# mhalushka/miRge3.0

Hardware: AMD Instinct MI355X
Metric: M reads/s through full annotation cascade; per-class counts bit-exact vs ref (higher is better)
Workload: dtype u64

## Files before the change

### mirge3.0_amd/csrc/kernels_collapse.hpp

```cpp
#pragma once
template <int W>
__device__ __forceinline__ bool same_read(const GroupView<W>& g, uint32_t a, const MirgeRead<W>& r) {
    if (g.len[a] != (uint8_t)r.len) return false;
    bool eq = true;
#pragma unroll
    for (int w = 0; w < W; w++) {
        eq &= g.seq[(size_t)w * g.n + a] == r.w[w];
        if (g.nmask) eq &= g.nmask[(size_t)w * g.n + a] == r.nm[w];
    }
    return eq;
}

template <int W>
__global__ void k_collapse_insert(GroupView<W> g, uint32_t* __restrict__ rep, uint32_t* __restrict__ firstj,
                                  uint32_t* __restrict__ cnt, uint32_t* __restrict__ slot_of,
                                  uint32_t mask, const int32_t* __restrict__ sample_ids,
                                  const uint32_t* __restrict__ orig, uint32_t base, int32_t S, uint32_t j_lo, uint32_t j_hi,
                                  const uint32_t* __restrict__ weight) {
    __shared__ unsigned long long c_key[MIRGE_CELL_CACHE];
    __shared__ uint32_t c_min[MIRGE_CELL_CACHE];
    __shared__ uint32_t c_cnt[MIRGE_CELL_CACHE];
    for (uint32_t i = threadIdx.x; i < MIRGE_CELL_CACHE; i += blockDim.x) { c_key[i] = 0ull; c_min[i] = 0xFFFFFFFFu; c_cnt[i] = 0; }
    __syncthreads();
    for (uint32_t j = j_lo + blockIdx.x * blockDim.x + threadIdx.x; j < j_hi; j += gridDim.x * blockDim.x) {
// ... 4 lines not shown
        for (int w = 1; w < W; w++) h = mirge_mix64(h ^ r.w[w]);
#pragma unroll
        for (int w = 0; w < W; w++) h ^= mirge_mix64(r.nm[w] + 0x9e3779b97f4a7c15ull * (w + 1));
        uint32_t s = (uint32_t)(h >> 20) & mask;
        while (true) {
            uint32_t cur = rep[s];
            if (cur == MIRGE_EMPTY) cur = atomicCAS(&rep[s], MIRGE_EMPTY, j);
            if (cur == MIRGE_EMPTY || cur == j || same_read<W>(g, cur, r)) break;
            s = (s + 1) & mask;
        }
        slot_of[j] = s;
        const uint32_t hidx = orig ? orig[j] : base + j;
        const int32_t sid = sample_ids ? sample_ids[hidx] : 0;
        const uint32_t wgt = weight ? weight[hidx] : 1u;
        const unsigned long long cell = (unsigned long long)s * (unsigned)S + (unsigned)sid + 1ull;
        uint32_t cs = (uint32_t)(mirge_mix64(cell) >> 11) & (MIRGE_CELL_CACHE - 1);
        bool cached = false;
        for (int t = 0; t < 4; t++) {
            unsigned long long cur = c_key[cs];
            if (cur == 0ull) cur = atomicCAS(&c_key[cs], 0ull, cell);
            if (cur == 0ull || cur == cell) {
                atomicMin(&c_min[cs], j);
                atomicAdd(&c_cnt[cs], wgt);
                cached = true;
                break;
            }
            cs = (cs + 1) & (MIRGE_CELL_CACHE - 1);
        }
        if (!cached) {
            atomicMin(&firstj[s], j);
            atomicAdd(&cnt[(size_t)s * S + sid], wgt);
        }
    }
    __syncthreads();
    for (uint32_t i = threadIdx.x; i < MIRGE_CELL_CACHE; i += blockDim.x) {
        const unsigned long long cell = c_key[i];
        if (cell == 0ull) continue;
        const unsigned long long lin = cell - 1ull;
        atomicMin(&firstj[lin / (unsigned)S], c_min[i]);
        atomicAdd(&cnt[lin], c_cnt[i]);
    }
}

struct KeySlot {
    unsigned long long key;
    uint32_t first_inv;
    uint32_t cnt;
};

__global__ void k_collapse_insert_key(GroupView<1> g, KeySlot* __restrict__ slots, uint32_t* __restrict__ slot_of,
                                      uint32_t mask) {
    for (uint32_t j = blockIdx.x * blockDim.x + threadIdx.x; j < g.n; j += gridDim.x * blockDim.x) {
        const unsigned long long key = g.seq[j] | (1ull << (2 * g.len[j]));
        uint32_t s = (uint32_t)(mirge_mix64(key) >> 20) & mask;
        uint32_t seen_first = 0;
        while (true) {
            const uint4 v = *reinterpret_cast<const uint4*>(&slots[s]);
            unsigned long long cur = ((unsigned long long)v.y << 32) | v.x;
            seen_first = v.z;
            if (cur == 0ull) { cur = atomicCAS(&slots[s].key, 0ull, key); seen_first = 0; }
            if (cur == 0ull || cur == key) break;
            s = (s + 1) & mask;
        }
        slot_of[j] = s;
        if (0xFFFFFFFFu - j > seen_first) atomicMax(&slots[s].first_inv, 0xFFFFFFFFu - j);
        atomicAdd(&slots[s].cnt, 1u);
    }
}

__global__ void k_collapse_init(uint32_t* __restrict__ rep, uint32_t* __restrict__ firstj, uint32_t* __restrict__ cnt,
                                uint32_t tsize, uint64_t ncnt) {
    for (uint64_t i = blockIdx.x * (uint64_t)blockDim.x + threadIdx.x; i < ncnt; i += (uint64_t)gridDim.x * blockDim.x) {
        if (i < tsize) { rep[i] = MIRGE_EMPTY; firstj[i] = MIRGE_EMPTY; }
        cnt[i] = 0;
    }
}

#ifndef MIRGE_PART_CAP
#define MIRGE_PART_CAP 4096
#endif
#ifndef MIRGE_PART_B1
#define MIRGE_PART_B1 64
#endif
#ifndef MIRGE_PART_SMALL
#define MIRGE_DEDUP_SHARDS 8
#define MIRGE_DEDUP_SHARD_STRIDE 1024
#define MIRGE_PART_SMALL 1600
#endif
#ifndef MIRGE_PART_W2
#define MIRGE_PART_W2 4
#endif
#define MIRGE_PART_MAXREG 256

__device__ __forceinline__ unsigned long long read_key64(const GroupView<1>& g, uint32_t j) {
    return g.seq[j] | (1ull << (2 * g.len[j]));
}

__device__ __forceinline__ uint32_t region_of(const uint32_t* pre, uint32_t R, uint32_t i, uint32_t& within) {
    uint32_t lo = 0, hi = R;
    while (lo < hi) {
        const uint32_t mid = (lo + hi) >> 1;
        if (pre[mid] > i) hi = mid; else lo = mid + 1;
    }
    within = i - (lo ? pre[lo - 1] : 0u);
    return lo;
}

__device__ __forceinline__ uint32_t region_prefix(const uint32_t* __restrict__ cnt, uint32_t R, uint32_t cap, uint32_t* pre) {
    for (uint32_t r = threadIdx.x; r < R; r += blockDim.x) pre[r] = min(cnt[r], cap);
    __syncthreads();
    if (threadIdx.x == 0) {
        uint32_t run = 0;
        for (uint32_t r = 0; r < R; r++) { run += pre[r]; pre[r] = run; }
    }
    __syncthreads();
    return R ? pre[R - 1] : 0u;
}

#ifndef MIRGE_PART_THREADS
#define MIRGE_PART_THREADS 1024
#endif
#ifndef MIRGE_AGG_BUCKET4
#define MIRGE_AGG_BUCKET4 1
#endif
#ifndef MIRGE_AGG_UNROLL
#define MIRGE_AGG_UNROLL 2
#endif
__global__ void __launch_bounds__(MIRGE_PART_THREADS)
k_part_agg(GroupView<1> g, const uint32_t* __restrict__ orig, uint32_t base, uint32_t chunk, uint32_t shift1, uint32_t NB1,
           uint32_t bshift, uint32_t B, uint32_t CS, uint32_t cap1, uint4* __restrict__ rec1, uint32_t* __restrict__ cnt1,
           uint32_t* __restrict__ hist, uint32_t* __restrict__ overflow, uint32_t* __restrict__ n_records, uint32_t* __restrict__ shard_cur) {
    if (shard_cur && blockIdx.x == 0 && threadIdx.x < MIRGE_DEDUP_SHARDS) shard_cur[threadIdx.x * MIRGE_DEDUP_SHARD_STRIDE] = 0u;
    extern __shared__ __attribute__((aligned(16))) unsigned long long lds_a[];
    uint32_t* c_min = reinterpret_cast<uint32_t*>(lds_a + CS);
    uint32_t* c_cnt = c_min + CS;
    uint32_t* cur = c_cnt + CS;
    uint32_t* lds_h = cur + NB1;
    for (uint32_t i = threadIdx.x; i < CS; i += blockDim.x) { lds_a[i] = 0ull; c_min[i] = 0xFFFFFFFFu; c_cnt[i] = 0; }
    for (uint32_t b = threadIdx.x; b < NB1; b += blockDim.x) cur[b] = 0;
    if (hist) for (uint32_t b = threadIdx.x; b < B; b += blockDim.x) lds_h[b] = 0;
    __syncthreads();
    const uint32_t lo = blockIdx.x * chunk, hi = min(lo + chunk, g.n);
    const uint32_t G = gridDim.x;
    auto append = [&](unsigned long long key, uint64_t h, uint32_t jr, uint32_t count) {
        const uint32_t b1 = (uint32_t)(h >> shift1);
        const uint32_t p = atomicAdd(&cur[b1], 1u);
        if (p < cap1) {
            rec1[((size_t)b1 * G + blockIdx.x) * cap1 + p] = make_uint4((uint32_t)key, (uint32_t)(key >> 32), jr, count);
            if (hist) atomicAdd(&lds_h[(uint32_t)(h >> bshift)], 1u);
        }
    };
    for (uint32_t j0 = lo; j0 < hi; j0 += blockDim.x * MIRGE_AGG_UNROLL) {
        unsigned long long keys[MIRGE_AGG_UNROLL];
        uint32_t jrs[MIRGE_AGG_UNROLL];
#pragma unroll
        for (int u = 0; u < MIRGE_AGG_UNROLL; u++) {
            const uint32_t j = j0 + u * blockDim.x + threadIdx.x;
            keys[u] = 0ull; jrs[u] = 0;
            if (j < hi) {
                keys[u] = read_key64(g, j);
                jrs[u] = orig ? orig[j] : base + j;
            }
        }
#pragma unroll
        for (int u = 0; u < MIRGE_AGG_UNROLL; u++) {
        const uint32_t j = j0 + u * blockDim.x + threadIdx.x;
        bool direct = false;
        unsigned long long key = keys[u];
        uint32_t jr = jrs[u];
        uint64_t h = 0;
        if (j < hi) {
            h = mirge_mix64(key);
            direct = true;
#if MIRGE_AGG_BUCKET4
            const uint32_t b0 = ((uint32_t)(h >> 9) & (CS / 4 - 1)) * 4;
            const ulonglong2 ka = *reinterpret_cast<const ulonglong2*>(&lds_a[b0]);
            const ulonglong2 kb = *reinterpret_cast<const ulonglong2*>(&lds_a[b0 + 2]);
            const unsigned long long k4[4] = {ka.x, ka.y, kb.x, kb.y};
            int slot = -1;
#pragma unroll
            for (int t = 0; t < 4; t++) if (slot < 0 && k4[t] == key) slot = t;
            if (slot < 0) {
#pragma unroll
                for (int t = 0; t < 4; t++) {
                    if (slot >= 0 || k4[t] != 0ull) continue;
                    const unsigned long long c0 = atomicCAS(&lds_a[b0 + t], 0ull, key);
                    if (c0 == 0ull || c0 == key) slot = t;
                }
            }
            if (slot >= 0) {
                const uint32_t s = b0 + (uint32_t)slot;
                if (*(volatile uint32_t*)&c_min[s] > jr) atomicMin(&c_min[s], jr);
                atomicAdd(&c_cnt[s], 1u);
                direct = false;
            }
#else
            uint32_t s = (uint32_t)(h >> 9) & (CS - 1);
            for (int t = 0; t < 4; t++) {
                unsigned long long c0 = lds_a[s];
                if (c0 == 0ull) c0 = atomicCAS(&lds_a[s], 0ull, key);
                if (c0 == 0ull || c0 == key) {
                    if (*(volatile uint32_t*)&c_min[s] > jr) atomicMin(&c_min[s], jr);
                    atomicAdd(&c_cnt[s], 1u);
                    direct = false;
                    break;
                }
                s = (s + 1) & (CS - 1);
            }
#endif
        }
        uint32_t count = 1;
        bool open = direct;
#pragma unroll
        for (int round = 0; round < 2; round++) {
            const unsigned long long ob = __ballot(open);
            if (!ob) break;
            const int lead = __ffsll(ob) - 1;
            const unsigned long long k0 = __shfl(key, lead, 64);
            const bool same = open && key == k0;
            const unsigned long long sb = __ballot(same);
            if (__popcll(sb) > 1) {
                uint32_t mn = same ? jr : 0xFFFFFFFFu;
#pragma unroll
                for (int o = 32; o > 0; o >>= 1) mn = min(mn, (uint32_t)__shfl_xor((int)mn, o, 64));
                if ((threadIdx.x & 63) == lead) { jr = mn; count = (uint32_t)__popcll(sb); }
                else if (same) direct = false;
            }
            open = open && !same;
        }
        if (direct) append(key, h, jr, count);
        }
    }
    __syncthreads();
    for (uint32_t i = threadIdx.x; i < CS; i += blockDim.x) {
        const unsigned long long key = lds_a[i];
        if (key != 0ull) append(key, mirge_mix64(key), c_min[i], c_cnt[i]);
    }
    __syncthreads();
    for (uint32_t b = threadIdx.x; b < NB1; b += blockDim.x) {
        const uint32_t n = cur[b];
        cnt1[(size_t)b * G + blockIdx.x] = min(n, cap1);
        if (n > cap1) atomicOr(overflow, 1u);
    }
    if (threadIdx.x == 0) {
        uint32_t mine = 0;
        for (uint32_t b = 0; b < NB1; b++) mine += min(cur[b], cap1);
        atomicAdd(n_records, mine);
    }
    if (hist) for (uint32_t b = threadIdx.x; b < B; b += blockDim.x) hist[(size_t)blockIdx.x * B + b] = lds_h[b];
}

__global__ void __launch_bounds__(MIRGE_PART_THREADS)
k_part_split(const uint4* __restrict__ rec1, const uint32_t* __restrict__ cnt1, const uint32_t* __restrict__ hist, uint32_t G,
             uint32_t B, uint32_t cap1, uint32_t W2, uint32_t RPW, uint32_t shift2, uint32_t NB2, uint64_t slab,
             uint4* __restrict__ rec2, uint32_t* __restrict__ off2, uint32_t* __restrict__ cnt2) {
    extern __shared__ __attribute__((aligned(16))) uint32_t lds_s[];
    uint32_t* pre = lds_s;
    uint32_t* cur = lds_s + MIRGE_PART_MAXREG;
    __shared__ uint32_t scan_tmp[MIRGE_PART_THREADS / 64 + 1];
    const uint32_t b1 = blockIdx.x / W2, w = blockIdx.x % W2;
    const uint32_t r0 = w * RPW, R = r0 < G ? min(RPW, G - r0) : 0u;
    uint32_t mine = 0;
    if (threadIdx.x < NB2)
        for (uint32_t r = 0; r < R; r++) mine += hist[(size_t)(r0 + r) * B + (size_t)b1 * NB2 + threadIdx.x];
    uint32_t tot_all;
    const uint32_t off = block_excl_scan<MIRGE_PART_THREADS / 64>(mine, tot_all, scan_tmp);
    if (threadIdx.x < NB2) {
        cur[threadIdx.x] = off;
        const size_t cell = ((size_t)b1 * NB2 + threadIdx.x) * W2 + w;
        off2[cell] = off;
        cnt2[cell] = mine;
    }
    for (uint32_t r = threadIdx.x; r < R; r += blockDim.x) pre[r] = min(cnt1[(size_t)b1 * G + r0 + r], cap1);
    __syncthreads();
    const uint4* in = rec1 + ((size_t)b1 * G + r0) * cap1;
    uint4* out = rec2 + (size_t)blockIdx.x * slab;
    const uint32_t wave = threadIdx.x >> 6, lane = threadIdx.x & 63, n_waves = blockDim.x >> 6;
    for (uint32_t r = wave; r < R; r += n_waves) {
        const uint32_t n = pre[r];
        const uint4* src = in + (size_t)r * cap1;
        for (uint32_t i0 = lane; i0 < n; i0 += 256) {
            uint4 rec[4];
#pragma unroll
            for (int u = 0; u < 4; u++)
                if (i0 + 64 * u < n) rec[u] = src[i0 + 64 * u];
#pragma unroll
            for (int u = 0; u < 4; u++) {
                if (i0 + 64 * u >= n) continue;
                const unsigned long long key = ((unsigned long long)rec[u].y << 32) | rec[u].x;
                const uint32_t b2 = (uint32_t)(mirge_mix64(key) >> shift2) & (NB2 - 1);
                out[atomicAdd(&cur[b2], 1u)] = rec[u];
            }
        }
    }
}

#ifndef MIRGE_DEDUP_K
#define MIRGE_DEDUP_K 2
#endif
#ifndef MIRGE_DEDUP_DEPTH
#define MIRGE_DEDUP_DEPTH 2
#endif

struct DedupShares {
    uint32_t e0, e1, e2, total, o0, o1, o2, o3;
    size_t base;
};
__device__ __forceinline__ DedupShares dedup_shares(uint32_t co, uint32_t cap32, size_t base) {
    DedupShares s;
    s.e0 = min((uint32_t)__builtin_amdgcn_readlane((int)co, 0), cap32);
    s.e1 = s.e0 + min((uint32_t)__builtin_amdgcn_readlane((int)co, 1), cap32);
    s.e2 = s.e1 + min((uint32_t)__builtin_amdgcn_readlane((int)co, 2), cap32);
    s.total = s.e2 + min((uint32_t)__builtin_amdgcn_readlane((int)co, 3), cap32);
    s.o0 = (uint32_t)__builtin_amdgcn_readlane((int)co, 4);
    s.o1 = (uint32_t)__builtin_amdgcn_readlane((int)co, 5);
    s.o2 = (uint32_t)__builtin_amdgcn_readlane((int)co, 6);
    s.o3 = (uint32_t)__builtin_amdgcn_readlane((int)co, 7);
    s.base = base;
    return s;
}
__device__ __forceinline__ size_t dedup_record_at(const DedupShares& s, uint64_t rcap, uint32_t i) {
    return s.base + (i < s.e0 ? (size_t)s.o0 + i : i < s.e1 ? rcap + s.o1 + (i - s.e0) : i < s.e2 ? 2 * rcap + s.o2 + (i - s.e1) : 3 * rcap + s.o3 + (i - s.e2));
}

#ifndef MIRGE_DEDUP_THREADS
#define MIRGE_DEDUP_THREADS 512
#endif
template <int CAP, bool FEW>
__global__ void __launch_bounds__(MIRGE_DEDUP_THREADS) __attribute__((amdgpu_waves_per_eu(CAP <= 2048 ? 8 : 4)))
k_part_dedup(const uint4* __restrict__ rec, const uint32_t* __restrict__ cnt, const uint32_t* __restrict__ off, uint32_t R,
             uint64_t rcap, uint32_t NB2, uint32_t B, uint64_t* __restrict__ useq, uint8_t* __restrict__ ulen,
             uint32_t* __restrict__ ucnt, uint32_t* __restrict__ ufirst, uint32_t* __restrict__ cursor,
             uint32_t* __restrict__ hist, uint32_t* __restrict__ overflow, uint32_t* __restrict__ shard_cur_in, uint32_t shard_cap,
             const uint32_t* __restrict__ n_records, uint32_t rec_thresh, uint64_t* __restrict__ sseq, uint8_t* __restrict__ slen, uint32_t* __restrict__ scnt,
             uint32_t* __restrict__ sfirst) {
    constexpr int T = MIRGE_DEDUP_THREADS, PER = CAP / T, K = MIRGE_DEDUP_K, D = MIRGE_DEDUP_DEPTH;
    static_assert(PER % 4 == 0 && K >= 2 && D >= 1, "a thread reads its slots out with 16-byte LDS operations");
    uint32_t lane_zero = 0u;
    asm volatile("" : "+v"(lane_zero));
    uint32_t n_rec_now = 0u;
    if (threadIdx.x == 0 && shard_cur_in) n_rec_now = n_records[lane_zero];
    extern __shared__ __attribute__((aligned(16))) unsigned long long lds_k[];
    uint32_t* lds_min = reinterpret_cast<uint32_t*>(lds_k + CAP);
    uint32_t* lds_cnt = lds_min + CAP;
    uint32_t* lds_x = lds_cnt + CAP;
    uint32_t* pre = lds_x + 64;
    uint32_t* roff = pre + MIRGE_PART_MAXREG;
    uint32_t& n_distinct = lds_x[0];
    {
        uint4* k4 = reinterpret_cast<uint4*>(lds_k);
        for (uint32_t i = threadIdx.x; i < CAP / 2; i += T) k4[i] = make_uint4(0u, 0u, 0u, 0u);
        uint4* m4 = reinterpret_cast<uint4*>(lds_min);
        for (uint32_t i = threadIdx.x; i < CAP / 4; i += T) m4[i] = make_uint4(~0u, ~0u, ~0u, ~0u);
        uint4* c4 = reinterpret_cast<uint4*>(lds_cnt);
        for (uint32_t i = threadIdx.x; i < CAP / 4; i += T) c4[i] = make_uint4(0u, 0u, 0u, 0u);
    }
    for (uint32_t i = threadIdx.x; i < 32 + 32; i += T)
        if (i != 18) lds_x[i] = 0;
    const uint32_t cap32 = (uint32_t)min(rcap, (uint64_t)0xFFFFFFFFu);
    const uint32_t grid = gridDim.x;
    uint32_t tid = threadIdx.x;

    auto insert = [&](const uint4 rc, const bool counted) {
        const unsigned long long key = ((unsigned long long)rc.y << 32) | rc.x;
        const uint32_t j = rc.z;
        uint32_t s = (uint32_t)(mirge_mix64(key) >> 7) & (CAP - 1);
        while (true) {
            unsigned long long c0 = lds_k[s];
            if (c0 == 0ull) {
                c0 = atomicCAS(&lds_k[s], 0ull, key);
                if (counted && c0 == 0ull && atomicAdd(&n_distinct, 1u) >= CAP - 64) atomicOr(overflow, 1u);
            }
            if (c0 == 0ull || c0 == key) break;
            if (counted && *(volatile uint32_t*)&n_distinct >= CAP - 32) break;
            s = (s + 1) & (CAP - 1);
        }
        if (*(volatile uint32_t*)&lds_min[s] > j) atomicMin(&lds_min[s], j);
        atomicAdd(&lds_cnt[s], rc.w);
    };
    struct ReadOut {
        unsigned long long key[PER];
        uint32_t mn[PER], ct[PER];
    };
    ReadOut ro[K];
    static_assert(K * 16 <= 32 && CAP <= 65536, "a thread's K ranks share one register");
    uint32_t ranks = 0u, tot[K];
    auto read_out = [&](ReadOut& o, uint32_t& rk, uint32_t& total) {
        const uint32_t s0 = tid * PER;
        uint32_t mine = 0, zero = 0u;
        asm volatile("" : "+v"(zero));
        const uint32_t ones = ~zero;
#pragma unroll
        for (int p = 0; p < PER; p += 2) {
            ulonglong2* at = reinterpret_cast<ulonglong2*>(&lds_k[s0 + p]);
            const ulonglong2 k2 = *at;
            *at = make_ulonglong2((unsigned long long)zero, (unsigned long long)zero);
            o.key[p] = k2.x; o.key[p + 1] = k2.y;
            mine += (k2.x != 0ull) + (k2.y != 0ull);
        }
#pragma unroll
        for (int p = 0; p < PER; p += 4) {
            uint4* am = reinterpret_cast<uint4*>(&lds_min[s0 + p]);
            uint4* ac = reinterpret_cast<uint4*>(&lds_cnt[s0 + p]);
            const uint4 m = *am, c = *ac;
            *am = make_uint4(ones, ones, ones, ones);
            *ac = make_uint4(zero, zero, zero, zero);
            o.mn[p] = m.x; o.mn[p + 1] = m.y; o.mn[p + 2] = m.z; o.mn[p + 3] = m.w;
            o.ct[p] = c.x; o.ct[p + 1] = c.y; o.ct[p + 2] = c.z; o.ct[p + 3] = c.w;
        }
        if (tid == 0) n_distinct = 0u;
        rk = block_excl_scan<T / 64>(mine, total, lds_x + 2, tid);
        total = (uint32_t)__builtin_amdgcn_readfirstlane((int)total);
    };
    const uint32_t* shard_cur = nullptr;
    uint32_t res_total = 0u, res_x = 0u, n_groups = 0u;
    auto reserve = [&](uint32_t& res_o, uint32_t total) {
        res_total = total;
        res_x = (blockIdx.x + n_groups++) % MIRGE_DEDUP_SHARDS;
        if (tid == 8 && total) res_o = shard_cur ? atomicAdd(&shard_cur_in[res_x * MIRGE_DEDUP_SHARD_STRIDE], total) : atomicAdd(cursor, total);
    };
    auto publish_base = [&](uint32_t res_o) {
        if (tid == 8) {
            uint32_t at = 0;
            if (res_total) {
                if (shard_cur) {
                    if (res_o + res_total > shard_cap) { atomicOr(overflow, 1u); at = 0xFFFFFFFFu; }
                    else at = res_x * shard_cap + res_o;
                } else at = res_o;
            }
            lds_x[1] = at;
        }
    };
    auto publish_mode = [&]() { if (tid == 0) lds_x[18] = (shard_cur_in && n_rec_now < rec_thresh) ? 1u : 0u; };
    auto take_mode = [&]() {
        if (__builtin_amdgcn_readfirstlane((int)lds_x[18])) { shard_cur = shard_cur_in; useq = sseq; ulen = slen; ucnt = scnt; ufirst = sfirst; }
    };
    auto emit = [&](const ReadOut& o, uint32_t r) {
#pragma unroll
        for (int p = 0; p < PER; p++) {
            const unsigned long long key = o.key[p];
            if (key == 0ull) continue;
            const int L = (63 - __clzll((long long)key)) >> 1;
            useq[r] = key ^ (1ull << (2 * L));
            ulen[r] = (uint8_t)L;
            ucnt[r] = o.ct[p];
// ... 249 lines not shown
```

### mirge3.0_amd/csrc/native_collapse.hpp

```cpp
#pragma once
struct CollapseTmp {
    uint32_t *rep = nullptr, *firstj = nullptr, *cnt = nullptr, *slot_of = nullptr, *blocksum = nullptr;
    KeySlot* slots = nullptr;
    uint8_t* flag = nullptr;
    const uint32_t* cnt_base = nullptr;
    uint32_t cnt_stride = 1, nb = 0;
    bool partitioned = false;
    uint4 *rec1 = nullptr, *rec2 = nullptr;
    uint32_t *cnt1 = nullptr, *cnt2 = nullptr, *off2 = nullptr, *hist = nullptr;
    uint32_t *shard_cur = nullptr, shard_cap = 0, *s_cnt = nullptr, *s_first = nullptr, rec_thresh = 0;
    uint64_t* s_seq = nullptr;
    uint8_t* s_len = nullptr;
    uint32_t G = 0, B = 0, NB1 = 0, NB2 = 1, W2 = 1, RPW = 0, cap1 = 0, shift2 = 0, cap = MIRGE_PART_CAP;
    uint64_t slab = 0;
};
#ifndef MIRGE_PART_CACHE
#define MIRGE_PART_CACHE 4096
#endif
#ifndef MIRGE_PART_RETRY_BYTES
#define MIRGE_PART_RETRY_BYTES (64ull << 30)
#endif
#define MIRGE_META_OVERFLOW 10
#define MIRGE_META_LONG_BASES 12
#define MIRGE_META_HIST 16
#define MIRGE_META_RECORDS (((MIRGE_META_HIST + MIRGE_MAX_READ_LEN + 1 + 63) & ~63) + 64)
#define MIRGE_META_WORDS (MIRGE_META_RECORDS + 64)

static const char* group_tag(int gi) {
    static const char* t[MIRGE_NGROUPS] = {".w1", ".w2", ".w4", ".w8", ".wl", ".w1n", ".w2n", ".w4n", ".w8n", ".wln"};
    return t[gi];
}

static uint32_t part_region_cap(double mean) {
    const double c = 1.25 * mean + 8.0 * std::sqrt(mean) + 64.0;
    return ((uint32_t)c + 3u) & ~3u;
}

static void part_len_hist(mirge_ctx* c, const ReadGroup& out, const CollapseTmp& t, uint32_t* dmeta, int gi) {
    if (!t.partitioned || !out.len) return;
    hipStream_t const was = c->cur;
    c->cur = c->aux;
    {
        LaunchScope ls(c, "k_len_hist", 0.0);
        hipLaunchKernelGGL(k_len_hist, dim3((unsigned)c->n_cu * 2), dim3(256), 0, c->aux, (const uint8_t*)out.len, (const uint32_t*)(dmeta + gi),
                           dmeta + MIRGE_META_HIST);
    }
    c->cur = was;
}

static int collapse_part_rest(mirge_ctx* c, int gi, const ReadGroup& in, ReadGroup& out, CollapseTmp& t, uint32_t* dmeta, int part = 0) {
    const bool two = t.NB2 > 1;
    if (part != 2 && two) {
        LaunchScope ls(c, "k_part_split.w1", in.n);
        hipLaunchKernelGGL(k_part_split, dim3(t.NB1 * t.W2), dim3(MIRGE_PART_THREADS), (MIRGE_PART_MAXREG + t.NB2) * 4, c->cur,
                           t.rec1, t.cnt1, t.hist, t.G, t.B, t.cap1, t.W2, t.RPW, t.shift2, t.NB2, t.slab, t.rec2, t.off2, t.cnt2);
    }
    if (part != 1) {
        LaunchScope ls(c, "k_part_dedup.w1", in.n);
        const uint4* rec = two ? t.rec2 : t.rec1;
        const uint32_t* cnt = two ? t.cnt2 : t.cnt1;
        const uint32_t* off = two ? t.off2 : nullptr;
        const uint32_t R = two ? t.W2 : t.G;
        const uint64_t rcap = two ? t.slab : (uint64_t)t.cap1;
        const bool sh = t.shard_cur != nullptr;
        uint64_t* const oseq = reinterpret_cast<uint64_t*>(out.seq);
        uint8_t* const olen = reinterpret_cast<uint8_t*>(out.len);
        static const uint32_t grid_env = std::getenv("MIRGE_DEDUP_GRID") ? (uint32_t)std::max(1, std::atoi(std::getenv("MIRGE_DEDUP_GRID"))) : 0u;
        uint32_t grid = std::min<uint32_t>(t.B, (uint32_t)c->n_cu * (t.cap == 2048 ? 4u : 2u));
        if (grid_env) grid = std::min(grid, grid_env);
        auto launch = [&](auto kern, unsigned lds) {
            hipLaunchKernelGGL(kern, dim3(grid), dim3(MIRGE_DEDUP_THREADS), lds, c->cur, rec, cnt, off, R, rcap, t.NB2, t.B, oseq, olen, out.counts,
                               out.first, dmeta + gi, (uint32_t*)nullptr, dmeta + MIRGE_META_OVERFLOW, t.shard_cur, t.shard_cap,
                               (const uint32_t*)(dmeta + MIRGE_META_RECORDS), t.rec_thresh, t.s_seq, t.s_len, t.s_cnt, t.s_first);
        };
        if (t.cap == 2048) {
            if (R <= 4) launch(k_part_dedup<2048, true>, 2048 * 16 + 4096);
            else launch(k_part_dedup<2048, false>, 2048 * 16 + 4096);
        } else {
            if (R <= 4) launch(k_part_dedup<MIRGE_PART_CAP, true>, MIRGE_PART_CAP * 16 + 4096);
            else launch(k_part_dedup<MIRGE_PART_CAP, false>, MIRGE_PART_CAP * 16 + 4096);
        }
        if (sh) {
            LaunchScope ls2(c, "k_part_compact.w1", in.n);
            hipLaunchKernelGGL(k_part_compact, dim3((unsigned)c->n_cu * 8), dim3(256), 0, c->cur, (const uint32_t*)t.shard_cur, t.shard_cap,
                               (const uint64_t*)t.s_seq, (const uint8_t*)t.s_len, (const uint32_t*)t.s_cnt, (const uint32_t*)t.s_first,
                               oseq, olen, out.counts, out.first, dmeta + gi, (const uint32_t*)(dmeta + MIRGE_META_RECORDS), t.rec_thresh);
        }
    }
    return 0;
}

template <int W>
static int collapse_phase_a(mirge_ctx* c, int gi, const ReadGroup& in, ReadGroup& out, CollapseTmp& t,
                            const int32_t* dsample, int32_t S, uint32_t* dmeta, int attempt, int stage = 0,
                            const uint32_t* dweight = nullptr) {
    const bool force_atomic = attempt >= 2 || (attempt == 1 && (uint64_t)in.n * 2048ull > MIRGE_PART_RETRY_BYTES);
    if (!in.n) return 0;
    if (stage == 2 && t.partitioned) return collapse_part_rest(c, gi, in, out, t, dmeta, 2);
    const bool key_path = (W == 1) && !in.nmask && S == 1 && !dweight;
    const uint64_t need = key_path ? (uint64_t)in.n + in.n / 2 : 2ull * in.n;
    uint64_t tsize64 = 1024;
    while (tsize64 < need) tsize64 <<= 1;
    if (tsize64 > (1ull << 31)) return fail(-5, "collapse: a read group of " + std::to_string(in.n) + " reads needs a hash table beyond 2^31 slots");
    const uint32_t tsize = (uint32_t)tsize64;
    const uint32_t per_block = MIRGE_BLOCK * MIRGE_SCAN_ITEMS;
    t.nb = (in.n + per_block - 1) / per_block;
    GroupView<W> v = view_of<W>(in);
    char name[48];
    const uint32_t* first_base;
    uint32_t first_stride;
    if (key_path && !force_atomic && in.n >= 65536) {
        t.partitioned = true;
        uint32_t B = 64;
        static const bool small_part = std::getenv("MIRGE_TEST_SMALL_PART") != nullptr;
        while (!small_part && B < 32768 && (uint64_t)B * 2048 < in.n) B <<= 1;
        t.cap = (!small_part && (uint64_t)B * MIRGE_PART_SMALL >= in.n) ? 2048u : (uint32_t)MIRGE_PART_CAP;
        static const uint32_t nb1_env = std::getenv("MIRGE_PART_NB1") ? (uint32_t)std::max(1, std::min(256, std::atoi(std::getenv("MIRGE_PART_NB1")))) : 0u;
        const uint32_t nb1_cap = nb1_env ? nb1_env : B >= 32768 ? 256u : B >= 16384 ? 128u : (uint32_t)MIRGE_PART_B1;
        const uint32_t NB1 = std::min<uint32_t>(B, nb1_cap), NB2 = B / NB1;
        const uint32_t CS = B > 16384 ? 1024 : MIRGE_PART_CACHE;
        const int agg_lds = (int)(CS * 16 + NB1 * 4 + (NB2 > 1 ? B * 4 : 0) + 64);
        static std::mutex attr_mu;
        static std::vector<int> attr_done;
        {
            std::lock_guard<std::mutex> lk(attr_mu);
            if (std::find(attr_done.begin(), attr_done.end(), c->device) == attr_done.end()) {
                HIPOK(hipFuncSetAttribute(reinterpret_cast<const void*>(k_part_agg), hipFuncAttributeMaxDynamicSharedMemorySize,
                                          1024 * 16 + 256 * 4 + 32768 * 4 + 64));
                HIPOK(hipFuncSetAttribute(reinterpret_cast<const void*>(k_part_dedup<MIRGE_PART_CAP, true>),
                                          hipFuncAttributeMaxDynamicSharedMemorySize, MIRGE_PART_CAP * 16 + 4096));
                HIPOK(hipFuncSetAttribute(reinterpret_cast<const void*>(k_part_dedup<MIRGE_PART_CAP, false>),
                                          hipFuncAttributeMaxDynamicSharedMemorySize, MIRGE_PART_CAP * 16 + 4096));
                attr_done.push_back(c->device);
            }
        }
        int lg = 0; while ((1u << lg) < B) lg++;
        int lg1 = 0; while ((1u << lg1) < NB1) lg1++;
        const uint32_t G = std::min<uint32_t>(256, (in.n + 2047) / 2048);
        uint32_t chunk = (in.n + G - 1) / G;
        chunk = (chunk + MIRGE_BLOCK - 1) / MIRGE_BLOCK * MIRGE_BLOCK;
        const uint32_t shift1 = 64 - lg1, shift2 = 64 - lg;
        const uint32_t w2_want = std::max<uint32_t>(1, (uint32_t)MIRGE_PART_W2 * (uint32_t)MIRGE_PART_B1 / NB1);
        const uint32_t W2 = NB2 > 1 ? std::min<uint32_t>(w2_want, G) : 1, RPW = (G + W2 - 1) / W2;
        static const bool small_region = std::getenv("MIRGE_TEST_SMALL_REGION") != nullptr;
        const uint32_t cap1 = attempt == 1 ? chunk
                                           : small_region ? std::max<uint32_t>(4, chunk / NB1 / 2 & ~3u) : part_region_cap((double)chunk / NB1);
        const uint64_t slab = (uint64_t)RPW * cap1;
        static const bool part_oom = std::getenv("MIRGE_TEST_PART_OOM") != nullptr;
        if (part_oom && attempt == 1) return fail(-3, "hipMalloc: out of memory (MIRGE_TEST_PART_OOM)");
        CHECK(dalloc(c, &t.rec1, (size_t)NB1 * G * cap1));
        CHECK(dalloc(c, &t.cnt1, (size_t)NB1 * G));
        static const int sharded_env = std::getenv("MIRGE_DEDUP_SHARDED") ? std::atoi(std::getenv("MIRGE_DEDUP_SHARDED")) : -1;
        static const double rec_share = std::getenv("MIRGE_DEDUP_REC_SHARE") ? std::atof(std::getenv("MIRGE_DEDUP_REC_SHARE")) : 0.45;
        const bool sharded = sharded_env != 0;
        t.rec_thresh = sharded_env > 0 ? 0xFFFFFFFFu : (uint32_t)std::min<double>(4.0e9, rec_share * (double)in.n);
        if (sharded && attempt == 0 && !small_part) {
            t.shard_cap = in.n / MIRGE_DEDUP_SHARDS + in.n / (8 * MIRGE_DEDUP_SHARDS) + 65536u;
            const size_t sn = (size_t)t.shard_cap * MIRGE_DEDUP_SHARDS;
            CHECK(dalloc(c, &t.shard_cur, (size_t)MIRGE_DEDUP_SHARDS * MIRGE_DEDUP_SHARD_STRIDE));
            CHECK(dalloc(c, &t.s_seq, sn));
            CHECK(dalloc(c, &t.s_len, sn));
            CHECK(dalloc(c, &t.s_cnt, sn));
            CHECK(dalloc(c, &t.s_first, sn));
        }
        if (NB2 > 1) {
            CHECK(dalloc(c, &t.hist, (size_t)G * B));
            CHECK(dalloc(c, &t.rec2, (size_t)NB1 * W2 * slab));
            CHECK(dalloc(c, &t.cnt2, (size_t)B * W2));
            CHECK(dalloc(c, &t.off2, (size_t)B * W2));
        }
        out.W = 1;
        CHECK(dalloc(c, &out.seq, (size_t)in.n));
        CHECK(dalloc(c, &out.len, (size_t)in.n));
        CHECK(dalloc(c, &out.counts, (size_t)in.n));
        CHECK(dalloc(c, &out.first, (size_t)in.n));
        GroupView<1> v1 = view_of<1>(in);
        {
            LaunchScope ls(c, "k_part_agg.w1", in.n);
            hipLaunchKernelGGL(k_part_agg, dim3(G), dim3(MIRGE_PART_THREADS), agg_lds, c->cur, v1, in.orig, in.base, chunk, shift1, NB1,
                               shift2, B, CS, cap1, t.rec1, t.cnt1, t.hist, dmeta + MIRGE_META_OVERFLOW, dmeta + MIRGE_META_RECORDS, t.shard_cur);
        }
        t.G = G; t.B = B; t.NB1 = NB1; t.NB2 = NB2; t.W2 = W2; t.RPW = RPW; t.cap1 = cap1; t.slab = slab; t.shift2 = shift2;
        if (stage == 1) return collapse_part_rest(c, gi, in, out, t, dmeta, 1);
        return collapse_part_rest(c, gi, in, out, t, dmeta);
    }
    if (stage == 1) return 0;
    CHECK(dalloc(c, &t.slot_of, in.n));
    CHECK(dalloc(c, &t.flag, (size_t)t.nb * per_block));
    CHECK(dalloc(c, &t.blocksum, t.nb));
    if (key_path) {
        CHECK(dalloc(c, &t.slots, tsize));
        HIPOK(hipMemsetAsync(t.slots, 0, (size_t)tsize * sizeof(KeySlot), c->cur));
        LaunchScope ls(c, "k_collapse_insert_key.w1", in.n);
        hipLaunchKernelGGL(k_collapse_insert_key, dim3(grid_for(c, in.n)), dim3(MIRGE_BLOCK), 0, c->cur,
                           view_of<1>(in), t.slots, t.slot_of, tsize - 1);
        first_base = reinterpret_cast<const uint32_t*>(t.slots) + 2; first_stride = 4;
        t.cnt_base = reinterpret_cast<const uint32_t*>(t.slots) + 3; t.cnt_stride = 4;
    } else {
        CHECK(dalloc(c, &t.rep, tsize));
        CHECK(dalloc(c, &t.firstj, tsize));
        CHECK(dalloc(c, &t.cnt, (size_t)tsize * S));
        hipLaunchKernelGGL(k_collapse_init, dim3(grid_for(c, (size_t)tsize * S)), dim3(MIRGE_BLOCK), 0, c->cur, t.rep, t.firstj, t.cnt,
                           tsize, (uint64_t)tsize * (uint64_t)S);
        std::snprintf(name, sizeof(name), "k_collapse_insert%s", group_tag(gi));
        LaunchScope ls(c, name, in.n);
        static const int ins_per_cu = std::getenv("MIRGE_INSERT_WG_PER_CU") ? std::max(1, std::atoi(std::getenv("MIRGE_INSERT_WG_PER_CU"))) : 0;
        const int ins_grid = std::min(grid_for(c, in.n), c->n_cu * (ins_per_cu ? ins_per_cu : (in.n < (2u << 20) ? 8 : 2)));
        const uint32_t seed = std::min<uint32_t>(in.n, MIRGE_COLLAPSE_SEED);
        hipLaunchKernelGGL(k_collapse_insert<W>, dim3((seed + MIRGE_BLOCK - 1) / MIRGE_BLOCK), dim3(MIRGE_BLOCK), 0, c->cur,
                           v, t.rep, t.firstj, t.cnt, t.slot_of, tsize - 1, dsample, in.orig, in.base, S, 0u, seed, dweight);
        if (in.n > seed)
            hipLaunchKernelGGL(k_collapse_insert<W>, dim3(ins_grid), dim3(MIRGE_BLOCK), 0, c->cur,
                               v, t.rep, t.firstj, t.cnt, t.slot_of, tsize - 1, dsample, in.orig, in.base, S, seed, in.n, dweight);
        first_base = t.firstj; first_stride = 1;
        t.cnt_base = t.cnt; t.cnt_stride = (uint32_t)S;
    }
    {
        std::snprintf(name, sizeof(name), "k_heads_blocksum%s", group_tag(gi));
        LaunchScope ls(c, name, in.n);
        hipLaunchKernelGGL(k_heads_blocksum, dim3(t.nb), dim3(MIRGE_BLOCK), 0, c->cur, t.slot_of, first_base, first_stride,
                           key_path ? 1u : 0u, in.n, in.len, t.flag, t.blocksum, dmeta + MIRGE_META_HIST);
    }
    {
        LaunchScope ls(c, "k_scan_blocksums", t.nb);
        hipLaunchKernelGGL(k_scan_blocksums, dim3(1), dim3(MIRGE_BLOCK), 0, c->cur, t.blocksum, t.nb, dmeta + gi);
    }
    return 0;
}

template <int W>
static int collapse_phase_b(mirge_ctx* c, int gi, const ReadGroup& in, ReadGroup& out, CollapseTmp& t, int32_t S,
                            uint32_t U, uint32_t out_base, const uint32_t* dmeta) {
    out.W = W; out.n = U; out.base = out_base;
    if (in.n && !t.partitioned) {
        CHECK(dalloc(c, &out.seq, (size_t)W * U));
        CHECK(dalloc(c, &out.len, (size_t)U));
        if (in.nmask) CHECK(dalloc(c, &out.nmask, (size_t)W * U));
        CHECK(dalloc(c, &out.counts, (size_t)U * S));
        CHECK(dalloc(c, &out.first, (size_t)U));
        char name[48];
        std::snprintf(name, sizeof(name), "k_collapse_scatter%s", group_tag(gi));
        LaunchScope ls(c, name, in.n);
        hipLaunchKernelGGL(k_collapse_scatter<W>, dim3(t.nb), dim3(MIRGE_BLOCK), 0, c->cur, view_of<W>(in), t.slot_of,
                           t.flag, t.cnt_base, t.cnt_stride, t.blocksum, dmeta + gi, in.orig, in.base, S, out.seq,
                           out.len, out.nmask, out.counts, out.first);
    }
    return 0;
}

static int collapse_phase_a_long(mirge_ctx* c, int gi, const ReadGroup& in, CollapseTmp& t, const int32_t* dsample, int32_t S,
                                 uint32_t* dmeta, int stage, const uint32_t* dweight) {
    if (!in.n || stage == 1) return 0;
    uint64_t tsize64 = 1024;
    while (tsize64 < 2ull * in.n) tsize64 <<= 1;
    if (tsize64 > (1ull << 31)) return fail(-5, "collapse: a read group of " + std::to_string(in.n) + " reads needs a hash table beyond 2^31 slots");
    const uint32_t tsize = (uint32_t)tsize64;
    const uint32_t per_block = MIRGE_BLOCK * MIRGE_SCAN_ITEMS;
    t.nb = (in.n + per_block - 1) / per_block;
    CHECK(dalloc(c, &t.slot_of, in.n));
    CHECK(dalloc(c, &t.flag, (size_t)t.nb * per_block));
    CHECK(dalloc(c, &t.blocksum, t.nb));
    CHECK(dalloc(c, &t.rep, tsize));
    CHECK(dalloc(c, &t.firstj, tsize));
    CHECK(dalloc(c, &t.cnt, (size_t)tsize * S));
    hipLaunchKernelGGL(k_collapse_init, dim3(grid_for(c, (size_t)tsize * S)), dim3(MIRGE_BLOCK), 0, c->cur, t.rep, t.firstj, t.cnt,
                       tsize, (uint64_t)tsize * (uint64_t)S);
    const LongView v = long_view_of(in);
    char name[48];
    {
        std::snprintf(name, sizeof(name), "k_collapse_insert%s", group_tag(gi));
        LaunchScope ls(c, name, in.n);
        hipLaunchKernelGGL(k_collapse_insert_long, dim3(grid_for(c, in.n)), dim3(MIRGE_BLOCK), 0, c->cur, v, t.rep, t.firstj, t.cnt, t.slot_of,
                           tsize - 1, dsample, in.orig, in.base, S, dweight);
// ... 340 lines not shown
```

Before: 8754.

## Batch agg hash probes across unroll lanes and parallelize split histogram reduction

The partition aggregation kernel is restructured so that all unrolled reads are loaded, hashed and probed against the LDS bucket cache in batched phases. CAS attempts now run in wave-uniform rounds, and output-slot atomics and record stores are issued in separate passes, which exposes memory-level parallelism and cuts divergence. The split kernel spreads its histogram column reduction over all waves with LDS atomics instead of having one thread walk every row, and it separates slot reservation from stores, using dummy counters for invalid lanes. This raises register pressure and slightly increases LDS use, and it adds an env knob for the cache size.

After: 8759 (median of 2 runs). About the same (+0.1%).

```diff
diff --git a/mirge3.0_amd/csrc/kernels_collapse.hpp b/mirge3.0_amd/csrc/kernels_collapse.hpp
--- a/mirge3.0_amd/csrc/kernels_collapse.hpp
+++ b/mirge3.0_amd/csrc/kernels_collapse.hpp
@@ -180,83 +180,144 @@
     };
     for (uint32_t j0 = lo; j0 < hi; j0 += blockDim.x * MIRGE_AGG_UNROLL) {
         unsigned long long keys[MIRGE_AGG_UNROLL];
-        uint32_t jrs[MIRGE_AGG_UNROLL];
+        uint32_t jrs[MIRGE_AGG_UNROLL], counts[MIRGE_AGG_UNROLL];
+        uint64_t hs[MIRGE_AGG_UNROLL];
+        bool direct[MIRGE_AGG_UNROLL];
+        {
+            uint64_t sq[MIRGE_AGG_UNROLL];
+            uint8_t ln[MIRGE_AGG_UNROLL];
+#pragma unroll
+            for (int u = 0; u < MIRGE_AGG_UNROLL; u++) {
+                const uint32_t j = j0 + u * blockDim.x + threadIdx.x, jc = min(j, hi - 1);
+                direct[u] = j < hi;
+                counts[u] = 1;
+                sq[u] = g.seq[jc];
+                ln[u] = g.len[jc];
+            }
+            if (orig) {
+#pragma unroll
+                for (int u = 0; u < MIRGE_AGG_UNROLL; u++) jrs[u] = orig[min(j0 + u * blockDim.x + threadIdx.x, hi - 1)];
+            } else {
+#pragma unroll
+                for (int u = 0; u < MIRGE_AGG_UNROLL; u++) jrs[u] = base + j0 + u * blockDim.x + threadIdx.x;
+            }
+#pragma unroll
+            for (int u = 0; u < MIRGE_AGG_UNROLL; u++) {
+                keys[u] = direct[u] ? sq[u] | (1ull << (2 * ln[u])) : 0ull;
+                hs[u] = direct[u] ? mirge_mix64(keys[u]) : 0ull;
+            }
+        }
+#if MIRGE_AGG_BUCKET4
+        uint32_t b0[MIRGE_AGG_UNROLL], freem[MIRGE_AGG_UNROLL];
+        int slot[MIRGE_AGG_UNROLL];
+        {
+            ulonglong2 ka[MIRGE_AGG_UNROLL], kb[MIRGE_AGG_UNROLL];
+#pragma unroll
+            for (int u = 0; u < MIRGE_AGG_UNROLL; u++) {
+                b0[u] = ((uint32_t)(hs[u] >> 9) & (CS / 4 - 1)) * 4;
+                ka[u] = *reinterpret_cast<const ulonglong2*>(&lds_a[b0[u]]);
+                kb[u] = *reinterpret_cast<const ulonglong2*>(&lds_a[b0[u] + 2]);
+            }
+#pragma unroll
+            for (int u = 0; u < MIRGE_AGG_UNROLL; u++) {
+                const unsigned long long k4[4] = {ka[u].x, ka[u].y, kb[u].x, kb[u].y};
+                slot[u] = -1; freem[u] = 0;
+#pragma unroll
+                for (int t = 0; t < 4; t++) {
+                    if (direct[u] && slot[u] < 0 && k4[t] == keys[u]) slot[u] = t;
+                    if (k4[t] == 0ull) freem[u] |= 1u << t;
+                }
+                if (!direct[u] || slot[u] >= 0) freem[u] = 0;
+            }
+        }
+#pragma unroll 1
+        for (int round = 0; round < 4; round++) {
+            uint32_t pending = 0;
+#pragma unroll
+            for (int u = 0; u < MIRGE_AGG_UNROLL; u++) pending |= freem[u];
+            if (!__ballot(pending != 0)) break;
+            unsigned long long c0[MIRGE_AGG_UNROLL];
+#pragma unroll
+            for (int u = 0; u < MIRGE_AGG_UNROLL; u++) {
+                c0[u] = 0ull;
+                if (freem[u]) c0[u] = atomicCAS(&lds_a[b0[u] + (uint32_t)(__ffs((int)freem[u]) - 1)], 0ull, keys[u]);
+            }
+#pragma unroll
+            for (int u = 0; u < MIRGE_AGG_UNROLL; u++) {
+                if (!freem[u]) continue;
+                if (c0[u] == 0ull || c0[u] == keys[u]) { slot[u] = __ffs((int)freem[u]) - 1; freem[u] = 0; }
+                else freem[u] &= freem[u] - 1;
+            }
+        }
+        uint32_t seen[MIRGE_AGG_UNROLL];
 #pragma unroll
         for (int u = 0; u < MIRGE_AGG_UNROLL; u++) {
-            const uint32_t j = j0 + u * blockDim.x + threadIdx.x;
-            keys[u] = 0ull; jrs[u] = 0;
-            if (j < hi) {
-                keys[u] = read_key64(g, j);
-                jrs[u] = orig ? orig[j] : base + j;
-            }
+            seen[u] = 0;
+            if (slot[u] >= 0) seen[u] = __hip_atomic_load(&c_min[b0[u] + (uint32_t)slot[u]], __ATOMIC_RELAXED, __HIP_MEMORY_SCOPE_WORKGROUP);
         }
 #pragma unroll
         for (int u = 0; u < MIRGE_AGG_UNROLL; u++) {
-        const uint32_t j = j0 + u * blockDim.x + threadIdx.x;
-        bool direct = false;
-        unsigned long long key = keys[u];
-        uint32_t jr = jrs[u];
-        uint64_t h = 0;
-        if (j < hi) {
-            h = mirge_mix64(key);
-            direct = true;
-#if MIRGE_AGG_BUCKET4
-            const uint32_t b0 = ((uint32_t)(h >> 9) & (CS / 4 - 1)) * 4;
-            const ulonglong2 ka = *reinterpret_cast<const ulonglong2*>(&lds_a[b0]);
-            const ulonglong2 kb = *reinterpret_cast<const ulonglong2*>(&lds_a[b0 + 2]);
-            const unsigned long long k4[4] = {ka.x, ka.y, kb.x, kb.y};
-            int slot = -1;
-#pragma unroll
-            for (int t = 0; t < 4; t++) if (slot < 0 && k4[t] == key) slot = t;
-            if (slot < 0) {
-#pragma unroll
-                for (int t = 0; t < 4; t++) {
-                    if (slot >= 0 || k4[t] != 0ull) continue;
-                    const unsigned long long c0 = atomicCAS(&lds_a[b0 + t], 0ull, key);
-                    if (c0 == 0ull || c0 == key) slot = t;
-                }
-            }
-            if (slot >= 0) {
-                const uint32_t s = b0 + (uint32_t)slot;
-                if (*(volatile uint32_t*)&c_min[s] > jr) atomicMin(&c_min[s], jr);
-                atomicAdd(&c_cnt[s], 1u);
-                direct = false;
-            }
+            if (slot[u] < 0) continue;
+            const uint32_t s = b0[u] + (uint32_t)slot[u];
+            if (seen[u] > jrs[u]) atomicMin(&c_min[s], jrs[u]);
+            atomicAdd(&c_cnt[s], 1u);
+            direct[u] = false;
+        }
 #else
-            uint32_t s = (uint32_t)(h >> 9) & (CS - 1);
+#pragma unroll
+        for (int u = 0; u < MIRGE_AGG_UNROLL; u++) {
+            if (!direct[u]) continue;
+            uint32_t s = (uint32_t)(hs[u] >> 9) & (CS - 1);
             for (int t = 0; t < 4; t++) {
                 unsigned long long c0 = lds_a[s];
-                if (c0 == 0ull) c0 = atomicCAS(&lds_a[s], 0ull, key);
-                if (c0 == 0ull || c0 == key) {
-                    if (*(volatile uint32_t*)&c_min[s] > jr) atomicMin(&c_min[s], jr);
+                if (c0 == 0ull) c0 = atomicCAS(&lds_a[s], 0ull, keys[u]);
+                if (c0 == 0ull || c0 == keys[u]) {
+                    if (__hip_atomic_load(&c_min[s], __ATOMIC_RELAXED, __HIP_MEMORY_SCOPE_WORKGROUP) > jrs[u]) atomicMin(&c_min[s], jrs[u]);
                     atomicAdd(&c_cnt[s], 1u);
-                    direct = false;
+                    direct[u] = false;
                     break;
                 }
                 s = (s + 1) & (CS - 1);
             }
-#endif
-        }
-        uint32_t count = 1;
-        bool open = direct;
-#pragma unroll
-        for (int round = 0; round < 2; round++) {
-            const unsigned long long ob = __ballot(open);
-            if (!ob) break;
-            const int lead = __ffsll(ob) - 1;
-            const unsigned long long k0 = __shfl(key, lead, 64);
-            const bool same = open && key == k0;
-            const unsigned long long sb = __ballot(same);
-            if (__popcll(sb) > 1) {
-                uint32_t mn = same ? jr : 0xFFFFFFFFu;
-#pragma unroll
-                for (int o = 32; o > 0; o >>= 1) mn = min(mn, (uint32_t)__shfl_xor((int)mn, o, 64));
-                if ((threadIdx.x & 63) == lead) { jr = mn; count = (uint32_t)__popcll(sb); }
-                else if (same) direct = false;
-            }
-            open = open && !same;
-        }
-        if (direct) append(key, h, jr, count);
+        }
+#endif
+#pragma unroll
+        for (int u = 0; u < MIRGE_AGG_UNROLL; u++) {
+            bool open = direct[u];
+#pragma unroll
+            for (int round = 0; round < 2; round++) {
+                const unsigned long long ob = __ballot(open);
+                if (!ob) break;
+                const int lead = __ffsll(ob) - 1;
+                const unsigned long long k0 =
+                    ((unsigned long long)(uint32_t)__builtin_amdgcn_readlane((int)(uint32_t)(keys[u] >> 32), lead) << 32) |
+                    (uint32_t)__builtin_amdgcn_readlane((int)(uint32_t)keys[u], lead);
+                const bool same = open && keys[u] == k0;
+                const unsigned long long sb = __ballot(same);
+                if (__popcll(sb) > 1) {
+                    uint32_t mn = same ? jrs[u] : 0xFFFFFFFFu;
+#pragma unroll
+                    for (int o = 32; o > 0; o >>= 1) mn = min(mn, (uint32_t)__shfl_xor((int)mn, o, 64));
+                    const bool leads = (int)(threadIdx.x & 63) == lead;
+                    jrs[u] = leads ? mn : jrs[u];
+                    counts[u] = leads ? (uint32_t)__popcll(sb) : counts[u];
+                    direct[u] = direct[u] && (leads || !same);
+                }
+                open = open && !same;
+            }
+        }
+        uint32_t at[MIRGE_AGG_UNROLL];
+#pragma unroll
+        for (int u = 0; u < MIRGE_AGG_UNROLL; u++) {
+            at[u] = cap1;
+            if (direct[u]) at[u] = atomicAdd(&cur[(uint32_t)(hs[u] >> shift1)], 1u);
+        }
+#pragma unroll
+        for (int u = 0; u < MIRGE_AGG_UNROLL; u++) {
+            if (at[u] >= cap1) continue;
+            rec1[((size_t)(uint32_t)(hs[u] >> shift1) * G + blockIdx.x) * cap1 + at[u]] =
+                make_uint4((uint32_t)keys[u], (uint32_t)(keys[u] >> 32), jrs[u], counts[u]);
+            if (hist) atomicAdd(&lds_h[(uint32_t)(hs[u] >> bshift)], 1u);
         }
     }
     __syncthreads();
@@ -278,6 +339,9 @@
     if (hist) for (uint32_t b = threadIdx.x; b < B; b += blockDim.x) hist[(size_t)blockIdx.x * B + b] = lds_h[b];
 }
 
+#ifndef MIRGE_SPLIT_DEPTH
+#define MIRGE_SPLIT_DEPTH 4
+#endif
 __global__ void __launch_bounds__(MIRGE_PART_THREADS)
 k_part_split(const uint4* __restrict__ rec1, const uint32_t* __restrict__ cnt1, const uint32_t* __restrict__ hist, uint32_t G,
              uint32_t B, uint32_t cap1, uint32_t W2, uint32_t RPW, uint32_t shift2, uint32_t NB2, uint64_t slab,
@@ -288,9 +352,22 @@
     __shared__ uint32_t scan_tmp[MIRGE_PART_THREADS / 64 + 1];
     const uint32_t b1 = blockIdx.x / W2, w = blockIdx.x % W2;
     const uint32_t r0 = w * RPW, R = r0 < G ? min(RPW, G - r0) : 0u;
-    uint32_t mine = 0;
-    if (threadIdx.x < NB2)
-        for (uint32_t r = 0; r < R; r++) mine += hist[(size_t)(r0 + r) * B + (size_t)b1 * NB2 + threadIdx.x];
+    const uint32_t wave = threadIdx.x >> 6, lane = threadIdx.x & 63, n_waves = blockDim.x >> 6;
+    for (uint32_t b = threadIdx.x; b < NB2; b += blockDim.x) cur[b] = 0;
+    __syncthreads();
+    for (uint32_t b = lane; b < NB2; b += 64) {
+        const uint32_t* col = hist + (size_t)r0 * B + (size_t)b1 * NB2 + b;
+        uint32_t part = 0;
+        for (uint32_t r = wave; r < R; r += 4 * n_waves) {
+            uint32_t v[4];
+#pragma unroll
+            for (int k = 0; k < 4; k++) v[k] = r + k * n_waves < R ? col[(size_t)(r + k * n_waves) * B] : 0u;
+            part += v[0] + v[1] + v[2] + v[3];
+        }
+        if (part) atomicAdd(&cur[b], part);
+    }
+    __syncthreads();
+    const uint32_t mine = threadIdx.x < NB2 ? cur[threadIdx.x] : 0u;
     uint32_t tot_all;
     const uint32_t off = block_excl_scan<MIRGE_PART_THREADS / 64>(mine, tot_all, scan_tmp);
     if (threadIdx.x < NB2) {
@@ -303,22 +380,25 @@
     __syncthreads();
     const uint4* in = rec1 + ((size_t)b1 * G + r0) * cap1;
     uint4* out = rec2 + (size_t)blockIdx.x * slab;
-    const uint32_t wave = threadIdx.x >> 6, lane = threadIdx.x & 63, n_waves = blockDim.x >> 6;
     for (uint32_t r = wave; r < R; r += n_waves) {
         const uint32_t n = pre[r];
         const uint4* src = in + (size_t)r * cap1;
-        for (uint32_t i0 = lane; i0 < n; i0 += 256) {
-            uint4 rec[4];
-#pragma unroll
-            for (int u = 0; u < 4; u++)
-                if (i0 + 64 * u < n) rec[u] = src[i0 + 64 * u];
-#pragma unroll
-            for (int u = 0; u < 4; u++) {
-                if (i0 + 64 * u >= n) continue;
+        for (uint32_t i0 = lane; i0 < n; i0 += 64 * MIRGE_SPLIT_DEPTH) {
+            uint4 rec[MIRGE_SPLIT_DEPTH];
+            uint32_t at[MIRGE_SPLIT_DEPTH];
+#pragma unroll
+            for (int u = 0; u < MIRGE_SPLIT_DEPTH; u++)
+                rec[u] = i0 + 64 * u < n ? src[i0 + 64 * u] : make_uint4(0u, 0u, 0u, 0u);
+#pragma unroll
+            for (int u = 0; u < MIRGE_SPLIT_DEPTH; u++) {
+                const bool ok = i0 + 64 * u < n;
                 const unsigned long long key = ((unsigned long long)rec[u].y << 32) | rec[u].x;
                 const uint32_t b2 = (uint32_t)(mirge_mix64(key) >> shift2) & (NB2 - 1);
-                out[atomicAdd(&cur[b2], 1u)] = rec[u];
-            }
+                at[u] = atomicAdd(&cur[ok ? b2 : NB2 + lane], 1u);
+            }
+#pragma unroll
+            for (int u = 0; u < MIRGE_SPLIT_DEPTH; u++)
+                if (i0 + 64 * u < n) out[at[u]] = rec[u];
         }
     }
 }
diff --git a/mirge3.0_amd/csrc/native_collapse.hpp b/mirge3.0_amd/csrc/native_collapse.hpp
--- a/mirge3.0_amd/csrc/native_collapse.hpp
+++ b/mirge3.0_amd/csrc/native_collapse.hpp
@@ -52,7 +52,7 @@
     const bool two = t.NB2 > 1;
     if (part != 2 && two) {
         LaunchScope ls(c, "k_part_split.w1", in.n);
-        hipLaunchKernelGGL(k_part_split, dim3(t.NB1 * t.W2), dim3(MIRGE_PART_THREADS), (MIRGE_PART_MAXREG + t.NB2) * 4, c->cur,
+        hipLaunchKernelGGL(k_part_split, dim3(t.NB1 * t.W2), dim3(MIRGE_PART_THREADS), (MIRGE_PART_MAXREG + t.NB2 + 64) * 4, c->cur,
                            t.rec1, t.cnt1, t.hist, t.G, t.B, t.cap1, t.W2, t.RPW, t.shift2, t.NB2, t.slab, t.rec2, t.off2, t.cnt2);
     }
     if (part != 1) {
@@ -118,7 +118,9 @@
         static const uint32_t nb1_env = std::getenv("MIRGE_PART_NB1") ? (uint32_t)std::max(1, std::min(256, std::atoi(std::getenv("MIRGE_PART_NB1")))) : 0u;
         const uint32_t nb1_cap = nb1_env ? nb1_env : B >= 32768 ? 256u : B >= 16384 ? 128u : (uint32_t)MIRGE_PART_B1;
         const uint32_t NB1 = std::min<uint32_t>(B, nb1_cap), NB2 = B / NB1;
-        const uint32_t CS = B > 16384 ? 1024 : MIRGE_PART_CACHE;
+        static const uint32_t cs_env = std::getenv("MIRGE_AGG_CACHE") ? (uint32_t)std::max(64, std::min(1 << 30, std::atoi(std::getenv("MIRGE_AGG_CACHE")))) : 0u;
+        uint32_t CS = B > 16384 ? 1024 : MIRGE_PART_CACHE;
+        if (cs_env) { uint32_t p2 = 64; while (p2 * 2 <= cs_env) p2 <<= 1; CS = std::min(CS, p2); }
         const int agg_lds = (int)(CS * 16 + NB1 * 4 + (NB2 > 1 ? B * 4 : 0) + 64);
         static std::mutex attr_mu;
         static std::vector<int> attr_done;
```
